# wenet-e2e/wenet

Hardware: AMD Instinct MI355X
Metric: audio-seconds/sec (RTF^-1), 12L Conformer fbank80, ctc_prefix_beam_search (higher is better)
Workload: dtype f32 (feed-forward and subsampling-conv2 GEMMs: fp32 operands as three exact bf16 planes, six plane products on the bf16 matrix cores, f32 accumulate -- error <= the v_mfma_f32 kernel's, tests/test_gpu_x6.py; everything else v_mfma_f32)

## Files before the change

### wenet_amd/csrc/gemm_x6.hip

```cpp
#include "common.h"
#include "gemm_epilogue.h"
#include "kernels.h"
#include "x6.h"

namespace wn {

namespace {

typedef int i32x4 __attribute__((ext_vector_type(4)));
typedef int i32x2 __attribute__((ext_vector_type(2)));

constexpr int REC = X3_REC;
constexpr int TILE3 = X3_TILE;
constexpr int XBN = 256;

__global__ __launch_bounds__(256) void x6_split_kernel(const float* __restrict__ src, int R,
                                                       int K, int ld, char* __restrict__ dst) {
  const int tiles = (R + 31) >> 5, nkb = K >> 4;
  const int64_t idx = (int64_t)blockIdx.x * 256 + threadIdx.x;
  const int row_l = (int)(idx & 31), h = (int)((idx >> 5) & 1);
  const int64_t rest = idx >> 6;
  const int kb = (int)(rest % nkb), tile = (int)(rest / nkb);
  if (tile >= tiles) return;
  const int row = tile * 32 + row_l;
  f32x4 a = {0.f, 0.f, 0.f, 0.f}, b = a;
  if (row < R) {
    const float* s = src + (int64_t)row * ld + kb * 16 + h * 8;
    a = *reinterpret_cast<const f32x4*>(s);
    b = *reinterpret_cast<const f32x4*>(s + 4);
  }
  bf16x8 p0, p1, p2;
#pragma unroll
  for (int e = 0; e < 4; ++e) {
    const Split3 sa = split3(a[e]), sb = split3(b[e]);
    p0[e] = sa.h0; p1[e] = sa.h1; p2[e] = sa.h2;
    p0[4 + e] = sb.h0; p1[4 + e] = sb.h1; p2[4 + e] = sb.h2;
  }
  char* o = dst + ((int64_t)kb * tiles + tile) * TILE3 + h * 512 + row_l * 16;
  *reinterpret_cast<bf16x8*>(o) = p0;
  *reinterpret_cast<bf16x8*>(o + REC) = p1;
  *reinterpret_cast<bf16x8*>(o + 2 * REC) = p2;
}

__device__ unsigned long long g_x6_clk[8][8];

template <int BM, int EPI, int ACT, bool CONV = false, bool AF32 = false, int NW = 8>
__global__ __launch_bounds__(NW * 64, 2) void gemm_x6_kernel(X6Args p, int tiles_m, int tiles_n) {
  extern __shared__ __attribute__((aligned(16))) char smem_x[];
  typedef __attribute__((address_space(3))) void* lds_ptr;
  unsigned long long ck0 = 0, ck1 = 0, ck2 = 0, rt0 = 0;
  if (p.probe & 4) { ck0 = __builtin_readcyclecounter(); rt0 = __builtin_amdgcn_s_memrealtime(); }
  static_assert(NW == 8 || (NW == 4 && BM == 128), "4 waves: 128-row tiles");
  constexpr int TA = BM / 32 / (NW / 4);
  constexpr int A_TILE = AF32 ? 2048 : TILE3;
  constexpr int A_BYTES = (BM / 32) * A_TILE;
  constexpr int STAGE = A_BYTES + 8 * TILE3;
  constexpr int NP = STAGE / REC;
  constexpr int RING = NW == 4 ? 2 : BM == 128 ? 4 : 3;

  const int nblk = tiles_m * tiles_n;
  const int bid = xcd_block_order(blockIdx.x, nblk * p.ksplit);
  const int slice = bid / nblk, tb = bid - slice * nblk;
  constexpr int GM = 4;
  const int per_group = GM * tiles_n;
  const int grp = tb / per_group, in_grp = tb - grp * per_group;
  const int gm = min(GM, tiles_m - grp * GM);
  const int tm = grp * GM + in_grp % gm, tn = in_grp / gm;
  const int m0 = p.row0 + tm * BM, n0 = tn * XBN;

  const int tid = threadIdx.x, lane = tid & 63;
  const int wave = __builtin_amdgcn_readfirstlane(tid >> 6);
  __builtin_assume(wave >= 0 && wave < NW);
  const int wm = wave >> 2, wn = wave & 3;
  const int hi = lane >> 5, li = lane & 31;

  const int Ta = CONV ? p.a_tiles : (p.M + 31) >> 5, Tb = (p.N + 31) >> 5;
  const int nkb_all = p.K >> 4;
  const int nkb = nkb_all / p.ksplit, kb0 = slice * nkb;
  const int64_t slab_a = (int64_t)Ta * TILE3, slab_b = (int64_t)Tb * TILE3;
  const __amdgpu_buffer_rsrc_t ra32 = __builtin_amdgcn_make_buffer_rsrc(
      const_cast<float*>(p.A), 0, (int)min(p.a_bytes, (int64_t)0x7fffffff), 0x00020000);
  const unsigned vlane = (unsigned)lane * 16u;
  constexpr int NPA = (A_BYTES / REC + NW - 1) / NW;
  int pix[NPA];
  if (CONV || AF32) {
#pragma unroll
    for (int q = 0; q < NPA; ++q) {
      const int j = q * NW + wave;
      const int rl = AF32 ? (j >> 1) * 32 + (j & 1) * 16 + (lane >> 2) : (j / 3) * 32 + li;
      const int row = min(m0 + rl, p.M - 1);
      if (CONV) pix[q] = p.a_pix[row];
      else pix[q] = row * p.lda * 4 + (((lane & 3) ^ ((rl >> 2) & 3)) << 4);
    }
    asm volatile("s_waitcnt vmcnt(0)" ::: "memory");
#pragma unroll
    for (int q = 0; q < NPA; ++q) asm volatile("" : "+v"(pix[q]));
  }
  __amdgpu_buffer_rsrc_t d_ra = ra32, d_rb = ra32;
  int d_sa = 0, d_sb = 0, d_delta = 0;
  char* d_dst = smem_x;
  auto make_desc = [&](int g) {
    const int kb = kb0 + g;
    d_dst = smem_x + (g % RING) * STAGE;
    d_sa = (m0 >> 5) * TILE3; d_delta = 0;
    int ka = kb, kw = kb;
    if (CONV) {
      int tap = kb / p.conv_kbc;
      ka = kb - tap * p.conv_kbc;
      if (p.conv_taps > 0) { ka = kb / p.conv_taps; tap = kb - ka * p.conv_taps; }
      kw = tap * p.conv_kbc + ka;
      d_sa = AF32 ? ka * 64 : 0;
      d_delta = p.tap_delta[tap];
    } else if (AF32) {
      d_sa = kb * 64;
    }
    if (!AF32)
      d_ra = __builtin_amdgcn_make_buffer_rsrc(
          const_cast<char*>(reinterpret_cast<const char*>(p.A3)) + ka * slab_a, 0,
          (int)min(slab_a, (int64_t)0x7fffffff), 0x00020000);
    d_rb = __builtin_amdgcn_make_buffer_rsrc(
        const_cast<char*>(reinterpret_cast<const char*>(p.B3)) + kw * slab_b, 0,
        (int)min(slab_b, (int64_t)0x7fffffff), 0x00020000);
    d_sb = (n0 >> 5) * TILE3;
  };
  constexpr int NPW = (NP + NW - 1) / NW;
  auto issue_piece = [&](int q) {
#ifdef WN_ABLATION
    if (p.probe & 2) return;
#endif
    const int j = q * NW + wave;
    const int qa = q < NPA ? q : NPA - 1;
    if (j < A_BYTES / REC) {
      if (AF32) {
        unsigned vo = (unsigned)pix[qa];
        if (CONV) {
          const int rl = (j & 1) * 16 + (lane >> 2);
          vo = (unsigned)((pix[qa] + d_delta) * p.conv_kbc * 64 +
                          (((lane & 3) ^ ((rl >> 2) & 3)) << 4));
        }
        __builtin_amdgcn_raw_ptr_buffer_load_lds(d_ra, (lds_ptr)(d_dst + j * REC), 16, vo, d_sa, 0,
                                                 0);
      } else if (CONV) {
        const int P = pix[qa] + d_delta;
        const unsigned vo = (unsigned)(((P >> 5) * 3 + j % 3) * REC + hi * 512 + (P & 31) * 16);
        __builtin_amdgcn_raw_ptr_buffer_load_lds(d_ra, (lds_ptr)(d_dst + j * REC), 16, vo, d_sa, 0,
                                                 0);
      } else {
        __builtin_amdgcn_raw_ptr_buffer_load_lds(d_ra, (lds_ptr)(d_dst + j * REC), 16, vlane,
                                                 d_sa + j * REC, 0, 0);
      }
    } else if (j < NP)
      __builtin_amdgcn_raw_ptr_buffer_load_lds(d_rb, (lds_ptr)(d_dst + j * REC), 16, vlane,
                                               d_sb + (j - A_BYTES / REC) * REC, 0, 0);
  };
  auto issue = [&](int g) {
    make_desc(g);
#pragma unroll
    for (int q = 0; q < NPW; ++q) issue_piece(q);
  };

  struct FA { bf16x8 p[3]; };
  struct FB { bf16x8 p[2][3]; };
  auto loadA = [&](int g, int i) {
    FA f;
    if constexpr (AF32) {
      const char* st = smem_x + (g % RING) * STAGE + (wm * TA + i) * A_TILE + li * 64;
      const int fz = (li >> 2) & 3;
      const f32x4 u = *reinterpret_cast<const f32x4*>(st + (((2 * hi) ^ fz) << 4));
      const f32x4 v = *reinterpret_cast<const f32x4*>(st + (((2 * hi + 1) ^ fz) << 4));
#pragma unroll
      for (int e = 0; e < 4; ++e) {
        const Split3 su = split3(u[e]), sv = split3(v[e]);
        f.p[0][e] = su.h0; f.p[1][e] = su.h1; f.p[2][e] = su.h2;
        f.p[0][4 + e] = sv.h0; f.p[1][4 + e] = sv.h1; f.p[2][4 + e] = sv.h2;
      }
    } else {
      const char* st = smem_x + (g % RING) * STAGE + (wm * TA + i) * TILE3 + lane * 16;
#pragma unroll
      for (int q = 0; q < 3; ++q) f.p[q] = *reinterpret_cast<const bf16x8*>(st + q * REC);
    }
    return f;
  };
  auto loadB = [&](int g) {
    const char* st = smem_x + (g % RING) * STAGE + A_BYTES + (wn * 2) * TILE3 + lane * 16;
    FB f;
#pragma unroll
    for (int j = 0; j < 2; ++j)
#pragma unroll
      for (int q = 0; q < 3; ++q)
        f.p[j][q] = *reinterpret_cast<const bf16x8*>(st + j * TILE3 + q * REC);
    return f;
  };

  f32x16 acc[TA][2];
#pragma unroll
  for (int i = 0; i < TA; ++i)
#pragma unroll
    for (int j = 0; j < 2; ++j)
#pragma unroll
      for (int r = 0; r < 16; ++r) acc[i][j][r] = 0.f;

  auto mma = [&](const FA& a, const FB& b, int i, auto&& between) {
    constexpr int PB[6] = {2, 0, 1, 1, 0, 0}, PA[6] = {0, 2, 1, 0, 1, 0};
#ifdef WN_ABLATION
    if (p.probe & 1) {
      asm volatile("" :: "v"(a.p[0]), "v"(a.p[1]), "v"(a.p[2]));
#pragma unroll
      for (int j = 0; j < 2; ++j) asm volatile("" :: "v"(b.p[j][0]), "v"(b.p[j][1]), "v"(b.p[j][2]));
      return;
    }
#endif
#pragma unroll
    for (int q = 0; q < 6; ++q) {
#pragma unroll
      for (int j = 0; j < 2; ++j)
        acc[i][j] = __builtin_amdgcn_mfma_f32_32x32x16_bf16(b.p[j][PB[q]], a.p[PA[q]],
                                                            acc[i][j], 0, 0, 0);
      between(q);
    }
  };

  constexpr int BAR = TA - 2;
  const int npw = (NP - wave + NW - 1) / NW;
  auto wait_pieces = [&](int stages_in_flight) {
    switch (stages_in_flight * npw) {
      case 0: asm volatile("s_waitcnt vmcnt(0)" ::: "memory"); break;
      case 4: asm volatile("s_waitcnt vmcnt(4)" ::: "memory"); break;
      case 5: asm volatile("s_waitcnt vmcnt(5)" ::: "memory"); break;
      case 6: asm volatile("s_waitcnt vmcnt(6)" ::: "memory"); break;
      case 8: asm volatile("s_waitcnt vmcnt(8)" ::: "memory"); break;
      case 9: asm volatile("s_waitcnt vmcnt(9)" ::: "memory"); break;
      case 10: asm volatile("s_waitcnt vmcnt(10)" ::: "memory"); break;
      case 12: asm volatile("s_waitcnt vmcnt(12)" ::: "memory"); break;
      default: asm volatile("s_waitcnt vmcnt(15)" ::: "memory"); break;
    }
  };
#pragma unroll
  for (int g = 0; g < RING; ++g)
    if (g < nkb) issue(g);
  wait_pieces(min(nkb, RING) - 1);
  __builtin_amdgcn_s_barrier();
  FB fb = loadB(0);
  FA fa = loadA(0, 0);
  if (p.probe & 4) ck1 = __builtin_readcyclecounter();
  constexpr int NS = TA - 1 > 0 ? TA - 1 : 1;
  constexpr int PP = (NPW + NS - 1) / NS;
  bool dnext_ok = false;
  for (int g = 0; g < nkb; ++g) {
#pragma unroll
    for (int i = 0; i < TA; ++i) {
      FA na; FB nb;
      if (i + 1 < TA) na = loadA(g, i + 1);
      else if (g + 1 < nkb) { nb = loadB(g + 1); na = loadA(g + 1, 0); }
      const int slot = i > BAR ? i - BAR - 1 : i < BAR ? TA - 1 - BAR + i : -1;
      mma(fa, fb, i, [&](int q) {
        if (TA < 3 || slot < 0 || !dnext_ok) return;
#pragma unroll
        for (int r = 0; r < PP; ++r) {
          const int qq = PP <= 3 ? (r * 6) / PP + 1 : r;
          const int pc = slot * PP + r;
          if (q == qq && pc < NPW) issue_piece(pc);
        }
      });
      if (i == BAR) {
        asm volatile("s_waitcnt lgkmcnt(0)" ::: "memory");
        wait_pieces(max(0, min(nkb - 2 - g, RING - 2)));
        __builtin_amdgcn_s_barrier();
        if (TA < 3) {
          if (g + RING < nkb) issue(g + RING);
        } else {
          dnext_ok = g + RING < nkb;
          if (dnext_ok) make_desc(g + RING);
        }
      }
      if (i + 1 < TA) fa = na;
      else if (g + 1 < nkb) { fa = na; fb = nb; }
    }
  }

  if (p.probe & 4) ck2 = __builtin_readcyclecounter();
  const int Tm = Ta;
#pragma unroll
  for (int j = 0; j < 2; ++j) {
    const int cb = n0 + (wn * 2 + j) * 32;
    f32x4 bias4[4] = {};
    if (EPI != 1 && p.bias) {
#pragma unroll
      for (int g = 0; g < 4; ++g)
        bias4[g] = *reinterpret_cast<const f32x4*>(p.bias + min(cb + 8 * g + 4 * hi, p.N - 4));
    }
#pragma unroll
    for (int i = 0; i < TA; ++i) {
      const int row = m0 + (wm * TA + i) * 32 + li;
      f32x4 v[4];
#pragma unroll
      for (int g = 0; g < 4; ++g)
#pragma unroll
        for (int e = 0; e < 4; ++e) {
          float x = acc[i][j][4 * g + e] + bias4[g][e];
          if (EPI != 1) {
            if (ACT == ACT_SILU) x = silu_fast(x);
            if (ACT == ACT_RELU) x = fmaxf(x, 0.0f);
            if (ACT == ACT_GELU) x = 0.5f * x * (1.0f + erff(x * 0.70710678118654752f));
          }
          v[g][e] = x;
        }
      if constexpr (EPI == 2) {
        i32x2 q[3][4];
#pragma unroll
        for (int g = 0; g < 4; ++g) {
          bf16x4 h0, h1, h2;
#pragma unroll
          for (int e = 0; e < 4; ++e) {
            const Split3 sp = split3(v[g][e]);
            h0[e] = sp.h0; h1[e] = sp.h1; h2[e] = sp.h2;
          }
          q[0][g] = __builtin_bit_cast(i32x2, h0);
          q[1][g] = __builtin_bit_cast(i32x2, h1);
          q[2][g] = __builtin_bit_cast(i32x2, h2);
        }
#pragma unroll
        for (int pl = 0; pl < 3; ++pl)
#pragma unroll
          for (int d = 0; d < 2; ++d) {
            auto s0 = __builtin_amdgcn_permlane32_swap(q[pl][0][d], q[pl][2][d], false, false);
            auto s1 = __builtin_amdgcn_permlane32_swap(q[pl][1][d], q[pl][3][d], false, false);
            q[pl][0][d] = s0[0]; q[pl][2][d] = s0[1];
            q[pl][1][d] = s1[0]; q[pl][3][d] = s1[1];
          }
        const int tile_m = (m0 >> 5) + wm * TA + i;
        const int kbn = (cb >> 4) + hi;
        if (tile_m < Tm && cb + 16 * hi < p.N) {
          char* o = reinterpret_cast<char*>(p.C3) + ((int64_t)kbn * Tm + tile_m) * TILE3 + li * 16;
#pragma unroll
          for (int pl = 0; pl < 3; ++pl) {
            *reinterpret_cast<i32x4*>(o + pl * REC) =
                i32x4{q[pl][0][0], q[pl][0][1], q[pl][2][0], q[pl][2][1]};
            *reinterpret_cast<i32x4*>(o + pl * REC + 512) =
                i32x4{q[pl][1][0], q[pl][1][1], q[pl][3][0], q[pl][3][1]};
          }
        }
      } else {
        if (row >= p.M) continue;
        float* crow = EPI == 1 ? p.C + ((int64_t)slice * p.M + row) * p.N
                               : p.C + (int64_t)row * p.ldc;
        f32x4 rs[4] = {};
        if (EPI == 0 && p.resid) {
#pragma unroll
          for (int g = 0; g < 4; ++g)
            rs[g] = *reinterpret_cast<const f32x4*>(p.resid + (int64_t)row * p.ldr +
                                                    min(cb + 8 * g + 4 * hi, p.N - 4));
        }
#pragma unroll
        for (int g = 0; g < 4; ++g) {
          const int c = cb + 8 * g + 4 * hi;
          if (c >= p.N) continue;
          f32x4 o = v[g];
          if constexpr (EPI == 0) {
            o *= p.alpha;
            if (p.resid) o += rs[g];
          }
          *reinterpret_cast<f32x4*>(crow + c) = o;
        }
      }
    }
  }
  if (p.probe & 4) {
    asm volatile("s_waitcnt vmcnt(0)" ::: "memory");
    const unsigned long long ck3 = __builtin_readcyclecounter();
    const unsigned long long rt1 = __builtin_amdgcn_s_memrealtime();
    if (blockIdx.x == gridDim.x / 2 && lane == 0) {
      unsigned long long* o = g_x6_clk[wave & 7];
      o[0] = ck0; o[1] = ck1; o[2] = ck2; o[3] = ck3; o[4] = rt0; o[5] = rt1; o[6] = nkb;
    }
  }
}

template <int BM, int EPI, int ACT, bool CONV = false, bool AF32 = false, int NW = 8>
int launch_x6(const X6Args& a, hipStream_t s) {
  const int tiles_m = cdiv(a.M - a.row0, BM), tiles_n = cdiv(a.N, XBN);
  const size_t lds = (size_t)(NW == 4 ? 2 : BM == 128 ? 4 : 3) *
                     ((BM / 32) * (AF32 ? 2048 : TILE3) + 8 * TILE3);
  auto kern = gemm_x6_kernel<BM, EPI, ACT, CONV, AF32, NW>;
  WN_MAX_DYN_LDS(kern, lds);
  hipLaunchKernelGGL(kern, dim3(tiles_m * tiles_n * a.ksplit), dim3(NW * 64), lds, s, a, tiles_m,
                     tiles_n);
  WN_HIP(hipGetLastError());
  return 0;
}

template <int BM, int EPI, bool AF32 = false, int NW = 8>
int launch_x6_act(const X6Args& a, hipStream_t s) {
  if (EPI == 1) return launch_x6<BM, EPI, ACT_NONE, false, AF32, NW>(a, s);
  switch (a.act) {
    case ACT_NONE: return launch_x6<BM, EPI, ACT_NONE, false, AF32, NW>(a, s);
    case ACT_SILU: return launch_x6<BM, EPI, ACT_SILU, false, AF32, NW>(a, s);
    case ACT_RELU: return launch_x6<BM, EPI, ACT_RELU, false, AF32, NW>(a, s);
    case ACT_GELU: return launch_x6<BM, EPI, ACT_GELU, false, AF32, NW>(a, s);
    default: break;
  }
  set_error("gemm_x6: unsupported activation");
  return -1;
}

}


namespace {
__global__ __launch_bounds__(256) void conv_tail_reduce_kernel(const float* __restrict__ P, int S,
                                                               int rows, int N4,
                                                               const float* __restrict__ bias,
                                                               float* __restrict__ C, int ldc) {
  const int64_t i = (int64_t)blockIdx.x * 256 + threadIdx.x;
  if (i >= (int64_t)rows * N4) return;
  const int r = (int)(i / N4), c = (int)(i - (int64_t)r * N4) * 4;
  f32x4 acc = bias ? *reinterpret_cast<const f32x4*>(bias + c) : f32x4{0.f, 0.f, 0.f, 0.f};
  for (int sl = 0; sl < S; ++sl)
    acc += *reinterpret_cast<const f32x4*>(P + ((int64_t)sl * rows + r) * (N4 * 4) + c);
#pragma unroll
  for (int e = 0; e < 4; ++e) acc[e] = fmaxf(acc[e], 0.0f);
  *reinterpret_cast<f32x4*>(C + (int64_t)r * ldc + c) = acc;
}
}

int gemm_x6_clocks(unsigned long long* out) {
  WN_HIP(hipMemcpyFromSymbol(out, HIP_SYMBOL(g_x6_clk), sizeof(g_x6_clk)));
  return 0;
}

size_t x6_bytes(int R, int K) { return (size_t)(K / 16) * cdiv(R, 32) * TILE3; }

int x6_split(const float* src, int R, int K, int ld, void* dst, hipStream_t s) {
  WN_CHECK(src && dst && R > 0 && K > 0 && K % 16 == 0 && ld % 4 == 0, "x6_split: shape");
  const int64_t n = (int64_t)cdiv(R, 32) * (K / 16) * 64;
  hipLaunchKernelGGL(x6_split_kernel, dim3((unsigned)((n + 255) / 256)), dim3(256), 0, s, src, R,
                     K, ld, reinterpret_cast<char*>(dst));
  WN_HIP(hipGetLastError());
  return 0;
}

int gemm_x6_bm(int M, int N, int ksplit) {
  const int tn = cdiv(N, XBN) * ksplit;
  const int t256 = cdiv(M, 256) * tn, t128 = cdiv(M, 128) * tn;
  if (t256 < 512) return 128;
  const int rem = t128 % 512;
  const int half_rounds_128 = 2 * (t128 / 512) + (rem == 0 ? 0 : rem <= 256 ? 1 : 2);
  return half_rounds_128 < 2 * cdiv(t256, 256) ? 128 : 256;
}

int gemm_x6(const X6Args& args, hipStream_t s) {
  X6Args a = args;
  if (tune().x6_probe) a.probe = tune().x6_probe;
  const bool af32 = a.A != nullptr;
  WN_CHECK((a.A3 || af32) && a.B3 && a.M > 0 && a.N > 0 && a.K > 0 && a.K % 16 == 0,
           "gemm_x6: shape");
  WN_CHECK(a.ksplit >= 1 && (a.K / 16) % a.ksplit == 0, "gemm_x6: K split");
  WN_CHECK(a.N % 4 == 0 && (a.epi != 2 || a.N % 16 == 0), "gemm_x6: N");
  WN_CHECK((int64_t)cdiv(a.a_pix ? 32 * a.a_tiles : a.M, 32) * TILE3 < ((int64_t)1 << 31) &&
               (int64_t)cdiv(a.N, 32) * TILE3 < ((int64_t)1 << 31),
           "gemm_x6: a k-block slab of an operand image over 2 GB");
  WN_CHECK(!af32 || (a.a_bytes > 0 && a.a_bytes < ((int64_t)1 << 31) &&
                     (a.a_pix || a.lda % 4 == 0)), "gemm_x6: fp32 A operand");
  WN_CHECK(a.epi == 2 ? a.C3 != nullptr : a.C != nullptr, "gemm_x6: no output");
  WN_CHECK(a.epi == 1 || a.ksplit == 1, "gemm_x6: K slices need the partial epilogue");
  const int bm = a.bm ? a.bm : gemm_x6_bm(a.M, a.N, a.ksplit);
  if (a.a_pix) {
    WN_CHECK(a.epi == 0 && a.act == ACT_RELU && a.conv_kbc > 0 && (af32 || a.a_tiles > 0) &&
                 (a.K / 16) % a.conv_kbc == 0 && a.K / 16 / a.conv_kbc <= 9,
             "gemm_x6: gathered A operand");
    const int ncu = 256;
    const int t256 = cdiv(a.M, 256), full = t256 / ncu * ncu;
    auto run = [&](const X6Args& x, int rows) {
      if (af32) return rows == 256 ? launch_x6<256, 0, ACT_RELU, true, true>(x, s)
                                   : launch_x6<128, 0, ACT_RELU, true, true>(x, s);
      return rows == 256 ? launch_x6<256, 0, ACT_RELU, true>(x, s)
                         : launch_x6<128, 0, ACT_RELU, true, false, 4>(x, s);
    };
    if (a.bm == 0 && tune().x6_conv_bm == 128 && !af32) return run(a, 128);
    if (a.bm == 0 && a.N <= XBN && full > 0 && t256 - full > 0 && t256 - full <= ncu / 2) {
      X6Args main = a, rest = a;
      main.M = full * 256;
      rest.row0 = full * 256;
      if (run(main, 256) != 0) return -1;
      const int rem = t256 - full, nkb = a.K / 16;
      int S = 0;
      for (int t = std::min(4, ncu / rem); t >= 2; --t)
        if (nkb % t == 0) { S = t; break; }
      const int rows = a.M - full * 256;
      if (!af32 && S >= 2 && a.part &&
          a.part_bytes >= (size_t)S * rows * a.N * sizeof(float) && a.N % 4 == 0) {
        X6Args r = a;
        r.a_pix = a.a_pix + (size_t)full * 256;
        r.M = rows; r.row0 = 0; r.epi = 1; r.ksplit = S; r.C = a.part; r.bm = 256;
        if (launch_x6<256, 1, ACT_NONE, true>(r, s) != 0) return -1;
        const int64_t n4 = (int64_t)rows * (a.N / 4);
        hipLaunchKernelGGL(conv_tail_reduce_kernel, dim3((unsigned)((n4 + 255) / 256)), dim3(256),
                           0, s, a.part, S, rows, a.N / 4, a.bias,
                           a.C + (int64_t)full * 256 * a.ldc, a.ldc);
        WN_HIP(hipGetLastError());
        return 0;
      }
      return run(rest, 128);
    }
    return run(a, bm);
  }
#define WN_X6(BM, AF)                                          \
  switch (a.epi) {                                             \
    case 0: return launch_x6_act<BM, 0, AF>(a, s);             \
    case 1: return launch_x6_act<BM, 1, AF>(a, s);             \
    case 2: return launch_x6_act<BM, 2, AF>(a, s);             \
    default: break;                                            \
  }
  if (bm == 128 && !af32 && a.nw != 8) {
    switch (a.epi) {
      case 0: return launch_x6_act<128, 0, false, 4>(a, s);
      case 1: return launch_x6_act<128, 1, false, 4>(a, s);
      case 2: return launch_x6_act<128, 2, false, 4>(a, s);
      default: break;
    }
  } else if (af32) {
    if (bm == 256) { WN_X6(256, true) } else { WN_X6(128, true) }
  } else {
    if (bm == 256) { WN_X6(256, false) } else { WN_X6(128, false) }
  }
#undef WN_X6
  set_error("gemm_x6: unknown epilogue");
  return -1;
}

}
```

### wenet_amd/csrc/tune.h

```cpp
#pragma once
#include <stdint.h>

#include <string>

namespace wn {

#define WN_TUNE_KEYS(X)                                                                         \
                          \
  X(gemm_tile_bf16, 0)                                                                          \
                            \
  X(bf16_store, 1)                                                                              \
                      \
  X(lp_probe, 0)                                                                                \
                       \
  X(attn_split, 0)                                                                              \
                     \
  X(attn_bf16, 1)                                                                               \
                 \
  X(attn_bf16_nw, 0)                                                                            \
                                                                            \
  X(attn_bf16_defer, 80)                                                                        \
                                                              \
  X(attn_bf16_dma, 1)                                                                           \
                        \
  X(qkv_bf16, 1)                                                                                \
            \
  X(fp8_min_tiles, 192)                                                                         \
       \
  X(ffn_fused, 1)                                                                               \
                                                                   \
  X(gemm_x6, 1)                                                                                 \
                                         \
  X(x6_linear, 1)                                                                               \
                      \
  X(x6_af32, 0)                                                                                 \
            \
  X(x6_conv_af32, 0)                                                                            \
     \
  X(enc_gate_pos, 0)                                                                            \
                                                            \
  X(x6_conv_bm, 128)                                                                            \
                    \
  X(x6_probe, 0)                                                                                \
                     \
  X(ffn_x6f, 1)                                                                                 \
            \
  X(ffn_ximg, 1)                                                                                \
                             \
  X(ffn_x6f_ring, 3)                                                                            \
                  \
  X(ffn_x6f_var, 0)                                                                             \
                                                                        \
  X(x6r, 1)                                                                                     \
                  \
  X(x6r_chain, 1)                                                                               \
          \
  X(x6r_dwc, 1)                                                                                 \
        \
  X(x6r_pro, 1)                                                                                 \
            \
  X(x6r512_rows, 0)                                                                             \
                 \
  X(gemm_rowln, 1)                                                                              \
          \
  X(dwconv_tiled, 1)                                                                            \
                               \
  X(attn_x6, 1)                                                                                 \
                   \
  X(attn_xcd, 1)                                                                                \
        \
  X(attn_x6_galign, 2)                                                                          \
                             \
  X(attn_x6_order, 1)                                                                           \
    \
  X(attn_x6_var, 0)                                                                             \
        \
  X(attn_fold, 1)                                                                               \
                  \
  X(rescore_groups, 1)                                                                          \
                                                \
  X(rescore_prefetch, 1)                                                                        \
    \
  X(beam_weak_hash, 0)                                                                          \
                                                                              \
  X(beam_lds_pool, 1)                                                                           \
    \
  X(sync_spin, 1)                                                                               \
                         \
  X(ctc_wave, 1)                                                                                \
        \
  X(dec_skinny, 0)

struct Tune {
#define X(name, dflt) int name = dflt;
  WN_TUNE_KEYS(X)
#undef X
};

constexpr int32_t TUNE_INHERIT = INT32_MIN;

extern Tune g_tune_default;
extern thread_local const Tune* t_tune;
inline const Tune& tune() { return t_tune ? *t_tune : g_tune_default; }

int* tune_field(Tune& t, const std::string& key);
int tune_check(const std::string& key, int32_t value, const char* who);
void tune_resolve(const Tune& ovr, Tune* eff);
Tune tune_all_inherit();

}
```

Baseline: 72660.

## Add 16x16x32 bf16 MFMA path for x6 GEMM, default on conv GEMMs

Adds a templated M16 variant of the split-bf16 x6 GEMM kernel. It issues 16x16x32 bf16 MFMAs instead of 32x32x16, with matching LDS fragment loads, interleaved B-fragment prefetch and a rewritten epilogue that uses permlane16_swap to write plane images. A new tune key x6_mfma16 (default 2) enables it only for the subsampling-conv path (a_pix set), including the split-K tail. The smaller MFMA shape changes the instruction mix, latency and register pressure, and the added epilogue permutes and loads bring their own cost.

```diff
diff --git a/wenet_amd/csrc/gemm_x6.hip b/wenet_amd/csrc/gemm_x6.hip
--- a/wenet_amd/csrc/gemm_x6.hip
+++ b/wenet_amd/csrc/gemm_x6.hip
@@ -44,13 +44,15 @@
 
 __device__ unsigned long long g_x6_clk[8][8];
 
-template <int BM, int EPI, int ACT, bool CONV = false, bool AF32 = false, int NW = 8>
+template <int BM, int EPI, int ACT, bool CONV = false, bool AF32 = false, int NW = 8,
+          bool M16 = false>
 __global__ __launch_bounds__(NW * 64, 2) void gemm_x6_kernel(X6Args p, int tiles_m, int tiles_n) {
   extern __shared__ __attribute__((aligned(16))) char smem_x[];
   typedef __attribute__((address_space(3))) void* lds_ptr;
   unsigned long long ck0 = 0, ck1 = 0, ck2 = 0, rt0 = 0;
   if (p.probe & 4) { ck0 = __builtin_readcyclecounter(); rt0 = __builtin_amdgcn_s_memrealtime(); }
   static_assert(NW == 8 || (NW == 4 && BM == 128), "4 waves: 128-row tiles");
+  static_assert(!(M16 && AF32), "16x16x32 fragments are read from plane images");
   constexpr int TA = BM / 32 / (NW / 4);
   constexpr int A_TILE = AF32 ? 2048 : TILE3;
   constexpr int A_BYTES = (BM / 32) * A_TILE;
@@ -192,13 +194,49 @@
     return f;
   };
 
-  f32x16 acc[TA][2];
-#pragma unroll
-  for (int i = 0; i < TA; ++i)
+  struct GA { bf16x8 p[2][2]; };
+  struct GB { bf16x8 p[2][3]; };
+  const int l16 = lane & 15, q4 = lane >> 4;
+  auto frag_off = [&](int lo, int hi_) {
+    return (q4 < 2 ? lo : hi_) * REC + (q4 & 1) * 512 + l16 * 16;
+  };
+  const int o01 = frag_off(0, 1), o02 = frag_off(0, 2), o10 = frag_off(1, 0), o20 = frag_off(2, 0);
+  auto loadA16 = [&](int g, int i) {
+    const char* st = smem_x + (g % RING) * STAGE + (wm * TA + i) * TILE3;
+    GA f;
+#pragma unroll
+    for (int h = 0; h < 2; ++h) {
+      f.p[h][0] = *reinterpret_cast<const bf16x8*>(st + o01 + h * 256);
+      f.p[h][1] = *reinterpret_cast<const bf16x8*>(st + o02 + h * 256);
+    }
+    return f;
+  };
+  auto loadB16 = [&](int g, int j) {
+    const char* st = smem_x + (g % RING) * STAGE + A_BYTES + (wn * 2 + j) * TILE3;
+    GB f;
+#pragma unroll
+    for (int h = 0; h < 2; ++h) {
+      f.p[h][0] = *reinterpret_cast<const bf16x8*>(st + o01 + h * 256);
+      f.p[h][1] = *reinterpret_cast<const bf16x8*>(st + o10 + h * 256);
+      f.p[h][2] = *reinterpret_cast<const bf16x8*>(st + o20 + h * 256);
+    }
+    return f;
+  };
+
+  f32x16 acc[M16 ? 1 : TA][2];
+#pragma unroll
+  for (int i = 0; i < (M16 ? 1 : TA); ++i)
 #pragma unroll
     for (int j = 0; j < 2; ++j)
 #pragma unroll
       for (int r = 0; r < 16; ++r) acc[i][j][r] = 0.f;
+  f32x4 acc16[M16 ? TA : 1][2][2][2];
+#pragma unroll
+  for (int i = 0; i < (M16 ? TA : 1); ++i)
+#pragma unroll
+    for (int j = 0; j < 2; ++j)
+#pragma unroll
+      for (int r = 0; r < 16; ++r) acc16[i][j][r >> 3][(r >> 2) & 1][r & 3] = 0.f;
 
   auto mma = [&](const FA& a, const FB& b, int i, auto&& between) {
     constexpr int PB[6] = {2, 0, 1, 1, 0, 0}, PA[6] = {0, 2, 1, 0, 1, 0};
@@ -217,6 +255,20 @@
         acc[i][j] = __builtin_amdgcn_mfma_f32_32x32x16_bf16(b.p[j][PB[q]], a.p[PA[q]],
                                                             acc[i][j], 0, 0, 0);
       between(q);
+    }
+  };
+
+  auto mma16 = [&](const GA& a, const GB& b, int i, int j, auto&& between) {
+    constexpr int PW[3] = {2, 1, 0}, PA[3] = {1, 0, 0};
+#pragma unroll
+    for (int q = 0; q < 3; ++q) {
+#pragma unroll
+      for (int ha = 0; ha < 2; ++ha)
+#pragma unroll
+        for (int hw = 0; hw < 2; ++hw)
+          acc16[i][j][ha][hw] = __builtin_amdgcn_mfma_f32_16x16x32_bf16(
+              b.p[hw][PW[q]], a.p[ha][PA[q]], acc16[i][j][ha][hw], 0, 0, 0);
+      between(3 * j + q);
     }
   };
 
@@ -240,8 +292,10 @@
     if (g < nkb) issue(g);
   wait_pieces(min(nkb, RING) - 1);
   __builtin_amdgcn_s_barrier();
-  FB fb = loadB(0);
-  FA fa = loadA(0, 0);
+  FB fb; FA fa;
+  GB gb[2]; GA ga;
+  if constexpr (M16) { gb[0] = loadB16(0, 0); gb[1] = loadB16(0, 1); ga = loadA16(0, 0); }
+  else { fb = loadB(0); fa = loadA(0, 0); }
   if (p.probe & 4) ck1 = __builtin_readcyclecounter();
   constexpr int NS = TA - 1 > 0 ? TA - 1 : 1;
   constexpr int PP = (NPW + NS - 1) / NS;
@@ -249,11 +303,9 @@
   for (int g = 0; g < nkb; ++g) {
 #pragma unroll
     for (int i = 0; i < TA; ++i) {
-      FA na; FB nb;
-      if (i + 1 < TA) na = loadA(g, i + 1);
-      else if (g + 1 < nkb) { nb = loadB(g + 1); na = loadA(g + 1, 0); }
+      FA na; FB nb; GA nga;
       const int slot = i > BAR ? i - BAR - 1 : i < BAR ? TA - 1 - BAR + i : -1;
-      mma(fa, fb, i, [&](int q) {
+      auto between = [&](int q) {
         if (TA < 3 || slot < 0 || !dnext_ok) return;
 #pragma unroll
         for (int r = 0; r < PP; ++r) {
@@ -261,7 +313,20 @@
           const int pc = slot * PP + r;
           if (q == qq && pc < NPW) issue_piece(pc);
         }
-      });
+      };
+      if constexpr (M16) {
+        const bool next = i + 1 == TA && g + 1 < nkb;
+        if (i + 1 < TA) nga = loadA16(g, i + 1);
+        else if (next) nga = loadA16(g + 1, 0);
+        mma16(ga, gb[0], i, 0, between);
+        if (next) gb[0] = loadB16(g + 1, 0);
+        mma16(ga, gb[1], i, 1, between);
+        if (next) gb[1] = loadB16(g + 1, 1);
+      } else {
+      if (i + 1 < TA) na = loadA(g, i + 1);
+      else if (g + 1 < nkb) { nb = loadB(g + 1); na = loadA(g + 1, 0); }
+      mma(fa, fb, i, between);
+      }
       if (i == BAR) {
         asm volatile("s_waitcnt lgkmcnt(0)" ::: "memory");
         wait_pieces(max(0, min(nkb - 2 - g, RING - 2)));
@@ -273,13 +338,102 @@
           if (dnext_ok) make_desc(g + RING);
         }
       }
-      if (i + 1 < TA) fa = na;
-      else if (g + 1 < nkb) { fa = na; fb = nb; }
+      if constexpr (M16) {
+        if (i + 1 < TA || g + 1 < nkb) ga = nga;
+      } else {
+        if (i + 1 < TA) fa = na;
+        else if (g + 1 < nkb) { fa = na; fb = nb; }
+      }
     }
   }
 
   if (p.probe & 4) ck2 = __builtin_readcyclecounter();
   const int Tm = Ta;
+  if constexpr (M16) {
+#pragma unroll
+    for (int j = 0; j < 2; ++j) {
+      const int cb = n0 + (wn * 2 + j) * 32;
+      f32x4 bias4[2] = {};
+      if (EPI != 1 && p.bias) {
+#pragma unroll
+        for (int hw = 0; hw < 2; ++hw)
+          bias4[hw] = *reinterpret_cast<const f32x4*>(p.bias + min(cb + 16 * hw + 4 * q4, p.N - 4));
+      }
+#pragma unroll
+      for (int i = 0; i < TA; ++i)
+#pragma unroll
+        for (int ha = 0; ha < 2; ++ha) {
+          const int row = m0 + (wm * TA + i) * 32 + 16 * ha + l16;
+          f32x4 v[2];
+#pragma unroll
+          for (int hw = 0; hw < 2; ++hw)
+#pragma unroll
+            for (int e = 0; e < 4; ++e) {
+              float x = acc16[i][j][ha][hw][e] + bias4[hw][e];
+              if (EPI != 1) {
+                if (ACT == ACT_SILU) x = silu_fast(x);
+                if (ACT == ACT_RELU) x = fmaxf(x, 0.0f);
+                if (ACT == ACT_GELU) x = 0.5f * x * (1.0f + erff(x * 0.70710678118654752f));
+              }
+              v[hw][e] = x;
+            }
+          if constexpr (EPI == 2) {
+            i32x2 q[3][2];
+#pragma unroll
+            for (int hw = 0; hw < 2; ++hw) {
+              bf16x4 h0, h1, h2;
+#pragma unroll
+              for (int e = 0; e < 4; ++e) {
+                const Split3 sp = split3(v[hw][e]);
+                h0[e] = sp.h0; h1[e] = sp.h1; h2[e] = sp.h2;
+              }
+              q[0][hw] = __builtin_bit_cast(i32x2, h0);
+              q[1][hw] = __builtin_bit_cast(i32x2, h1);
+              q[2][hw] = __builtin_bit_cast(i32x2, h2);
+            }
+#pragma unroll
+            for (int pl = 0; pl < 3; ++pl)
+#pragma unroll
+              for (int d = 0; d < 2; ++d) {
+                auto sw = __builtin_amdgcn_permlane16_swap(q[pl][0][d], q[pl][1][d], false, false);
+                q[pl][0][d] = sw[0]; q[pl][1][d] = sw[1];
+              }
+            const int tile_m = (m0 >> 5) + wm * TA + i;
+            const int kbn = (cb >> 4) + (q4 & 1);
+            if (tile_m < Tm && cb + 16 * (q4 & 1) < p.N) {
+              char* o = reinterpret_cast<char*>(p.C3) + ((int64_t)kbn * Tm + tile_m) * TILE3 +
+                        (q4 >> 1) * 512 + (16 * ha + l16) * 16;
+#pragma unroll
+              for (int pl = 0; pl < 3; ++pl)
+                *reinterpret_cast<i32x4*>(o + pl * REC) =
+                    i32x4{q[pl][0][0], q[pl][0][1], q[pl][1][0], q[pl][1][1]};
+            }
+          } else {
+            if (row >= p.M) continue;
+            float* crow = EPI == 1 ? p.C + ((int64_t)slice * p.M + row) * p.N
+                                   : p.C + (int64_t)row * p.ldc;
+            f32x4 rs[2] = {};
+            if (EPI == 0 && p.resid) {
+#pragma unroll
+              for (int hw = 0; hw < 2; ++hw)
+                rs[hw] = *reinterpret_cast<const f32x4*>(p.resid + (int64_t)row * p.ldr +
+                                                         min(cb + 16 * hw + 4 * q4, p.N - 4));
+            }
+#pragma unroll
+            for (int hw = 0; hw < 2; ++hw) {
+              const int c = cb + 16 * hw + 4 * q4;
+              if (c >= p.N) continue;
+              f32x4 o = v[hw];
+              if constexpr (EPI == 0) {
+                o *= p.alpha;
+                if (p.resid) o += rs[hw];
+              }
+              *reinterpret_cast<f32x4*>(crow + c) = o;
+            }
+          }
+        }
+    }
+  } else {
 #pragma unroll
   for (int j = 0; j < 2; ++j) {
     const int cb = n0 + (wn * 2 + j) * 32;
@@ -365,6 +519,7 @@
       }
     }
   }
+  }
   if (p.probe & 4) {
     asm volatile("s_waitcnt vmcnt(0)" ::: "memory");
     const unsigned long long ck3 = __builtin_readcyclecounter();
@@ -376,12 +531,13 @@
   }
 }
 
-template <int BM, int EPI, int ACT, bool CONV = false, bool AF32 = false, int NW = 8>
+template <int BM, int EPI, int ACT, bool CONV = false, bool AF32 = false, int NW = 8,
+          bool M16 = false>
 int launch_x6(const X6Args& a, hipStream_t s) {
   const int tiles_m = cdiv(a.M - a.row0, BM), tiles_n = cdiv(a.N, XBN);
   const size_t lds = (size_t)(NW == 4 ? 2 : BM == 128 ? 4 : 3) *
                      ((BM / 32) * (AF32 ? 2048 : TILE3) + 8 * TILE3);
-  auto kern = gemm_x6_kernel<BM, EPI, ACT, CONV, AF32, NW>;
+  auto kern = gemm_x6_kernel<BM, EPI, ACT, CONV, AF32, NW, M16>;
   WN_MAX_DYN_LDS(kern, lds);
   hipLaunchKernelGGL(kern, dim3(tiles_m * tiles_n * a.ksplit), dim3(NW * 64), lds, s, a, tiles_m,
                      tiles_n);
@@ -389,14 +545,14 @@
   return 0;
 }
 
-template <int BM, int EPI, bool AF32 = false, int NW = 8>
+template <int BM, int EPI, bool AF32 = false, int NW = 8, bool M16 = false>
 int launch_x6_act(const X6Args& a, hipStream_t s) {
-  if (EPI == 1) return launch_x6<BM, EPI, ACT_NONE, false, AF32, NW>(a, s);
+  if (EPI == 1) return launch_x6<BM, EPI, ACT_NONE, false, AF32, NW, M16>(a, s);
   switch (a.act) {
-    case ACT_NONE: return launch_x6<BM, EPI, ACT_NONE, false, AF32, NW>(a, s);
-    case ACT_SILU: return launch_x6<BM, EPI, ACT_SILU, false, AF32, NW>(a, s);
-    case ACT_RELU: return launch_x6<BM, EPI, ACT_RELU, false, AF32, NW>(a, s);
-    case ACT_GELU: return launch_x6<BM, EPI, ACT_GELU, false, AF32, NW>(a, s);
+    case ACT_NONE: return launch_x6<BM, EPI, ACT_NONE, false, AF32, NW, M16>(a, s);
+    case ACT_SILU: return launch_x6<BM, EPI, ACT_SILU, false, AF32, NW, M16>(a, s);
+    case ACT_RELU: return launch_x6<BM, EPI, ACT_RELU, false, AF32, NW, M16>(a, s);
+    case ACT_GELU: return launch_x6<BM, EPI, ACT_GELU, false, AF32, NW, M16>(a, s);
     default: break;
   }
   set_error("gemm_x6: unsupported activation");
@@ -464,6 +620,8 @@
   WN_CHECK(a.epi == 2 ? a.C3 != nullptr : a.C != nullptr, "gemm_x6: no output");
   WN_CHECK(a.epi == 1 || a.ksplit == 1, "gemm_x6: K slices need the partial epilogue");
   const int bm = a.bm ? a.bm : gemm_x6_bm(a.M, a.N, a.ksplit);
+  const int k16 = tune().x6_mfma16;
+  const bool m16 = !af32 && (k16 == 1 || (k16 == 2 && a.a_pix != nullptr));
   if (a.a_pix) {
     WN_CHECK(a.epi == 0 && a.act == ACT_RELU && a.conv_kbc > 0 && (af32 || a.a_tiles > 0) &&
                  (a.K / 16) % a.conv_kbc == 0 && a.K / 16 / a.conv_kbc <= 9,
@@ -473,6 +631,8 @@
     auto run = [&](const X6Args& x, int rows) {
       if (af32) return rows == 256 ? launch_x6<256, 0, ACT_RELU, true, true>(x, s)
                                    : launch_x6<128, 0, ACT_RELU, true, true>(x, s);
+      if (m16) return rows == 256 ? launch_x6<256, 0, ACT_RELU, true, false, 8, true>(x, s)
+                                  : launch_x6<128, 0, ACT_RELU, true, false, 4, true>(x, s);
       return rows == 256 ? launch_x6<256, 0, ACT_RELU, true>(x, s)
                          : launch_x6<128, 0, ACT_RELU, true, false, 4>(x, s);
     };
@@ -492,7 +652,8 @@
         X6Args r = a;
         r.a_pix = a.a_pix + (size_t)full * 256;
         r.M = rows; r.row0 = 0; r.epi = 1; r.ksplit = S; r.C = a.part; r.bm = 256;
-        if (launch_x6<256, 1, ACT_NONE, true>(r, s) != 0) return -1;
+        if ((m16 ? launch_x6<256, 1, ACT_NONE, true, false, 8, true>(r, s)
+                 : launch_x6<256, 1, ACT_NONE, true>(r, s)) != 0) return -1;
         const int64_t n4 = (int64_t)rows * (a.N / 4);
         hipLaunchKernelGGL(conv_tail_reduce_kernel, dim3((unsigned)((n4 + 255) / 256)), dim3(256),
                            0, s, a.part, S, rows, a.N / 4, a.bias,
@@ -504,24 +665,21 @@
     }
     return run(a, bm);
   }
-#define WN_X6(BM, AF)                                          \
+#define WN_X6(BM, AF, NW, M16)                                 \
   switch (a.epi) {                                             \
-    case 0: return launch_x6_act<BM, 0, AF>(a, s);             \
-    case 1: return launch_x6_act<BM, 1, AF>(a, s);             \
-    case 2: return launch_x6_act<BM, 2, AF>(a, s);             \
+    case 0: return launch_x6_act<BM, 0, AF, NW, M16>(a, s);    \
+    case 1: return launch_x6_act<BM, 1, AF, NW, M16>(a, s);    \
+    case 2: return launch_x6_act<BM, 2, AF, NW, M16>(a, s);    \
     default: break;                                            \
   }
   if (bm == 128 && !af32 && a.nw != 8) {
-    switch (a.epi) {
-      case 0: return launch_x6_act<128, 0, false, 4>(a, s);
-      case 1: return launch_x6_act<128, 1, false, 4>(a, s);
-      case 2: return launch_x6_act<128, 2, false, 4>(a, s);
-      default: break;
-    }
+    if (m16) { WN_X6(128, false, 4, true) } else { WN_X6(128, false, 4, false) }
   } else if (af32) {
-    if (bm == 256) { WN_X6(256, true) } else { WN_X6(128, true) }
+    if (bm == 256) { WN_X6(256, true, 8, false) } else { WN_X6(128, true, 8, false) }
+  } else if (m16) {
+    if (bm == 256) { WN_X6(256, false, 8, true) } else { WN_X6(128, false, 8, true) }
   } else {
-    if (bm == 256) { WN_X6(256, false) } else { WN_X6(128, false) }
+    if (bm == 256) { WN_X6(256, false, 8, false) } else { WN_X6(128, false, 8, false) }
   }
 #undef WN_X6
   set_error("gemm_x6: unknown epilogue");
diff --git a/wenet_amd/csrc/tune.h b/wenet_amd/csrc/tune.h
--- a/wenet_amd/csrc/tune.h
+++ b/wenet_amd/csrc/tune.h
@@ -40,6 +40,8 @@
   X(enc_gate_pos, 0)                                                                            \
                                                             \
   X(x6_conv_bm, 128)                                                                            \
+    \
+  X(x6_mfma16, 2)                                                                               \
                     \
   X(x6_probe, 0)                                                                                \
                      \
```

Result: slower. 71470 (-1.6%).
